# gau-nernst/llama-x

Measured on AMD Instinct MI355X. Metric: train tokens/sec Llama-3.1-8B seq4096 at 1/2/4/8 MI355X; p50 step ms, higher is better.
Workload: dtype bf16; 1 GPU; Llama-3.1-8B text-only LoRA r=16 bf16, seq=4096, 1 sequence per GPU, causal mask, base+LM head frozen (BASELINE.json configs[1]); random-init weights at 8B dimensions; seq_len=4096, parallelism=dp1, launch=hipGraph replay (fwd+bwd+AdamW), lm_head_rows=labelled only

## Files before the change

### llama-x_amd/csrc/common.h

```cpp
#pragma once
#include <hip/hip_runtime.h>
#include <stdint.h>
#include <stdarg.h>
#include <stdio.h>

#define LLX_OK 0
#define LLX_ERR_ARG -1
#define LLX_ERR_LAUNCH -2
#define LLX_ERR_UNSUPPORTED -3

void llx_set_error(const char* fmt, ...);

#define LLX_REQUIRE(cond, ...)            \
  do {                                    \
    if (!(cond)) {                        \
      llx_set_error(__VA_ARGS__);         \
      return LLX_ERR_ARG;                 \
    }                                     \
  } while (0)

#define LLX_LAUNCH_CHECK(name)                                              \
  do {                                                                      \
    hipError_t e__ = hipGetLastError();                                     \
    if (e__ != hipSuccess) {                                                \
      llx_set_error("%s: launch failed: %s", name, hipGetErrorString(e__)); \
      return LLX_ERR_LAUNCH;                                                \
    }                                                                       \
  } while (0)

typedef uint16_t bf16_t;

typedef __attribute__((ext_vector_type(8))) __bf16 bf16x8_t;
typedef __attribute__((ext_vector_type(4))) float f32x4_t;
typedef __attribute__((ext_vector_type(16))) float f32x16_t;
typedef __attribute__((ext_vector_type(4))) int i32x4_t;
typedef __attribute__((ext_vector_type(16))) int i32x16_t;
typedef __attribute__((ext_vector_type(4))) short s16x4_t;
typedef __attribute__((ext_vector_type(4))) uint32_t u32x4_t;
typedef __attribute__((ext_vector_type(2))) uint32_t u32x2_t;

#define LLX_WAVE 64

__device__ __forceinline__ float bf2f(bf16_t v) { return __uint_as_float(((uint32_t)v) << 16); }
__device__ __forceinline__ bf16_t f2bf(float f) {
  __bf16 b = (__bf16)f;
  return __builtin_bit_cast(bf16_t, b);
}
__device__ __forceinline__ uint32_t pack_bf2(float lo, float hi) {
  return (uint32_t)f2bf(lo) | ((uint32_t)f2bf(hi) << 16);
}
__device__ __forceinline__ float bflo(uint32_t w) { return __uint_as_float(w << 16); }
__device__ __forceinline__ float bfhi(uint32_t w) { return __uint_as_float(w & 0xffff0000u); }

__device__ __forceinline__ float wave_sum(float v) {
#pragma unroll
  for (int o = 32; o > 0; o >>= 1) v += __shfl_xor(v, o, 64);
  return v;
}
__device__ __forceinline__ float wave_max(float v) {
#pragma unroll
  for (int o = 32; o > 0; o >>= 1) v = fmaxf(v, __shfl_xor(v, o, 64));
  return v;
}

__device__ __forceinline__ float block_sum(float v, float* red) {
  v = wave_sum(v);
  const int lane = threadIdx.x & 63, w = threadIdx.x >> 6, nw = (blockDim.x + 63) >> 6;
  __syncthreads();
  if (lane == 0) red[w] = v;
  __syncthreads();
  float t = 0.f;
  for (int i = 0; i < nw; ++i) t += red[i];
  return t;
}
__device__ __forceinline__ float block_max(float v, float* red) {
  v = wave_max(v);
  const int lane = threadIdx.x & 63, w = threadIdx.x >> 6, nw = (blockDim.x + 63) >> 6;
  __syncthreads();
  if (lane == 0) red[w] = v;
  __syncthreads();
  float t = red[0];
  for (int i = 1; i < nw; ++i) t = fmaxf(t, red[i]);
  return t;
}

static inline int64_t cdiv64(int64_t a, int64_t b) { return (a + b - 1) / b; }

__device__ __forceinline__ float q8_absmax8(const u32x4_t& v, float amax) {
#pragma unroll
  for (int e = 0; e < 4; ++e) amax = fmaxf(amax, fmaxf(fabsf(bflo(v[e])), fabsf(bfhi(v[e]))));
  return amax;
}
__device__ __forceinline__ float q8_scale(float amax) { return amax / 127.0f; }
__device__ __forceinline__ float q8_divisor(float scale) { return fmaxf(scale, 1e-12f); }
__device__ __forceinline__ u32x2_t q8_quant8(const u32x4_t& v, float div) {
  u32x2_t o = {0u, 0u};
#pragma unroll
  for (int e = 0; e < 4; ++e) {
    const int a = (int)rintf(bflo(v[e]) / div), b = (int)rintf(bfhi(v[e]) / div);
    o[e >> 1] |= ((uint32_t)(a & 0xff) | ((uint32_t)(b & 0xff) << 8)) << ((e & 1) * 16);
  }
  return o;
}

__device__ __forceinline__ float sigmoidf_(float x) { return __builtin_amdgcn_rcpf(1.f + __expf(-x)); }
__device__ __forceinline__ u32x4_t swiglu_fwd8(const u32x4_t& gv, const u32x4_t& uv) {
  u32x4_t o;
#pragma unroll
  for (int e = 0; e < 4; ++e) {
    const float g0 = bflo(gv[e]), g1 = bfhi(gv[e]);
    const float s0 = bf2f(f2bf(g0 * sigmoidf_(g0))), s1 = bf2f(f2bf(g1 * sigmoidf_(g1)));
    o[e] = pack_bf2(s0 * bflo(uv[e]), s1 * bfhi(uv[e]));
  }
  return o;
}
__device__ __forceinline__ void swiglu_bwd8(const u32x4_t& dv, const u32x4_t& gv, const u32x4_t& uv, u32x4_t& og, u32x4_t& ou) {
#pragma unroll
  for (int e = 0; e < 4; ++e) {
    float dgs[2], dus[2];
#pragma unroll
    for (int p = 0; p < 2; ++p) {
      const float gg = p ? bfhi(gv[e]) : bflo(gv[e]);
      const float uu = p ? bfhi(uv[e]) : bflo(uv[e]);
      const float dd = p ? bfhi(dv[e]) : bflo(dv[e]);
      const float sg = sigmoidf_(gg);
      const float silu = bf2f(f2bf(gg * sg));
      dus[p] = dd * silu;
      const float ds = bf2f(f2bf(dd * uu));
      dgs[p] = ds * (sg * (1.f + gg * (1.f - sg)));
    }
    og[e] = pack_bf2(dgs[0], dgs[1]);
    ou[e] = pack_bf2(dus[0], dus[1]);
  }
}

__device__ __forceinline__ u32x4_t rope8(const u32x4_t& v, const f32x4_t& t0, const f32x4_t& t1, float sign) {
  const float cs[4] = {t0[0], t0[2], t1[0], t1[2]};
  const float sn[4] = {t0[1] * sign, t0[3] * sign, t1[1] * sign, t1[3] * sign};
  u32x4_t o;
#pragma unroll
  for (int e = 0; e < 4; ++e) {
    const float x0 = bflo(v[e]), x1 = bfhi(v[e]);
    o[e] = pack_bf2(x0 * cs[e] - x1 * sn[e], x1 * cs[e] + x0 * sn[e]);
  }
  return o;
}

__device__ __forceinline__ u32x4_t rope8(const u32x4_t& v, const float* __restrict__ tp, float sign) {
  const f32x4_t t0 = *reinterpret_cast<const f32x4_t*>(tp);
  const f32x4_t t1 = *reinterpret_cast<const f32x4_t*>(tp + 4);
  const float cs[4] = {t0[0], t0[2], t1[0], t1[2]};
  const float sn[4] = {t0[1] * sign, t0[3] * sign, t1[1] * sign, t1[3] * sign};
  u32x4_t o;
#pragma unroll
  for (int e = 0; e < 4; ++e) {
    const float x0 = bflo(v[e]), x1 = bfhi(v[e]);
    o[e] = pack_bf2(x0 * cs[e] - x1 * sn[e], x1 * cs[e] + x0 * sn[e]);
  }
  return o;
}

typedef __attribute__((ext_vector_type(8))) short llx_s16x8_t;
template <int OFF>
__device__ __forceinline__ void lds_tr_read(s16x4_t& dst, uint32_t addr) {
  asm volatile("ds_read_b64_tr_b16 %0, %1 offset:%2" : "=v"(dst) : "v"(addr), "n"(OFF));
}
__device__ __forceinline__ void lds_tr_read_rt(s16x4_t& dst, uint32_t addr, int off) {
  asm volatile("ds_read_b64_tr_b16 %0, %1 offset:%2" : "=v"(dst) : "v"(addr), "n"(off));
}
template <int N>
__device__ __forceinline__ void lds_tr_wait4(s16x4_t& a, s16x4_t& b, s16x4_t& c, s16x4_t& d) {
  asm volatile("s_waitcnt lgkmcnt(%4)" : "+v"(a), "+v"(b), "+v"(c), "+v"(d) : "n"(N));
  __builtin_amdgcn_sched_barrier(0);
}
template <int N>
__device__ __forceinline__ void lds_tr_wait8(s16x4_t (&c)[4], s16x4_t (&d)[4]) {
  asm volatile("s_waitcnt lgkmcnt(%8)" : "+v"(c[0]), "+v"(c[1]), "+v"(c[2]), "+v"(c[3]), "+v"(d[0]), "+v"(d[1]), "+v"(d[2]), "+v"(d[3]) : "n"(N));
  __builtin_amdgcn_sched_barrier(0);
}
__device__ __forceinline__ void lds_read16_rt(i32x4_t& dst, uint32_t addr, int off) {
  asm volatile("ds_read_b128 %0, %1 offset:%2" : "=v"(dst) : "v"(addr), "n"(off));
}
template <typename T>
__device__ __forceinline__ void lds_pin1(T& x) { asm volatile("" : "+v"(x)); }
template <typename T, int N>
__device__ __forceinline__ void lds_pin1(T (&x)[N]) {
#pragma unroll
  for (int i = 0; i < N; ++i) asm volatile("" : "+v"(x[i]));
}
template <typename... T>
__device__ __forceinline__ void lds_pin(T&... x) {
  (lds_pin1(x), ...);
  __builtin_amdgcn_sched_barrier(0);
}
template <int N, typename... T>
__device__ __forceinline__ void lds_wait(T&... x) {
  asm volatile("s_waitcnt lgkmcnt(%0)" : : "n"(N));
  (lds_pin1(x), ...);
  __builtin_amdgcn_sched_barrier(0);
}
__device__ __forceinline__ bf16x8_t frag_of(const s16x4_t& lo, const s16x4_t& hi) {
  const llx_s16x8_t v = {lo[0], lo[1], lo[2], lo[3], hi[0], hi[1], hi[2], hi[3]};
// ... 11 lines not shown
```

### llama-x_amd/csrc/gemm_bf16.hip

```cpp
#include "common.h"
#include <type_traits>
#include <mutex>

#define BM 256
#define BN 256
#define BK 64
#define STAGE_BYTES (2 * 256 * BK * 2)
#define A_TILE_BYTES (256 * BK * 2)
#define EPI_ROW_BYTES 528
#define GEMM_LDS_BYTES (256 * EPI_ROW_BYTES)

enum { EPI_NONE = 0, EPI_RESIDUAL = 1, EPI_BIAS = 2, EPI_BIAS_GELU = 3, EPI_COLSCALE = 4, EPI_ROWCOLSCALE = 5, EPI_SWIGLU_BWD = 6, EPI_SWIGLU_FWD = 7, EPI_ROPE = 8, EPI_SPLITK = 9, EPI_ROWCOLSCALE_F32 = 10 };

struct GemmArgs {
  const bf16_t* A; const bf16_t* B; bf16_t* C;
  const bf16_t* A2; const bf16_t* B2;
  const bf16_t* E;
  const bf16_t* E2;
  int64_t lda, ldb, ldc, lde, lda2, ldb2;
  int M, N, K, K2;
  int grid_m, grid_n;
  int col0, col_end;
  const bf16_t* sa; const bf16_t* sb;
  const float* rope;
  int rope_S, rope_cols;
  const int* m_valid;
  float* C32;
  int splits;
};

typedef __attribute__((address_space(3))) void lds_void;
typedef const __attribute__((address_space(1))) void gbl_void;

__device__ __forceinline__ float gelu_erf(float x) { return 0.5f * x * (1.0f + erff(x * 0.70710678118654752440f)); }

template <int EPI, bool I8, int PIPE, int BNT = 256>
__global__ __launch_bounds__(512, 2) void gemm_nt_kernel(const GemmArgs g) {
  static_assert(BNT == 256 || BNT == 128, "tile width");
  static_assert(PIPE == 1, "the four-phase main loop is the only one");
  static_assert(BNT == 256 || EPI != EPI_SWIGLU_FWD, "the SwiGLU-forward epilogue needs the full tile");
  constexpr int ESZ = I8 ? 1 : 2;
  constexpr int TK = 128 / ESZ;
  constexpr int WNG = BNT / 64;
  constexpr int WR = 256 / (8 / WNG);
  constexpr int MI = WR / 16;
  constexpr int MH = MI / 2;
  constexpr int BSI = BNT / 64;
  constexpr int EROW = BNT * 2 + 16;
  extern __shared__ __attribute__((aligned(16))) char smem[];
  const int tid = threadIdx.x;
  const int lane = tid & 63;
  const int wave = __builtin_amdgcn_readfirstlane(tid >> 6);
  const int wm = wave / WNG, wn = wave % WNG;

  int grid_m = g.grid_m;
  if (g.m_valid != nullptr) grid_m = min(grid_m, (*g.m_valid + BM - 1) / BM);
  const int nsplit = EPI == EPI_SPLITK ? g.splits : 1;
  const int nwg = grid_m * g.grid_n * nsplit;
  int bid = blockIdx.x;
  if (bid >= nwg) return;
  {
    const int q = nwg >> 3, r = nwg & 7, x = bid & 7;
    bid = (x < r ? x * (q + 1) : r * (q + 1) + (x - r) * q) + (bid >> 3);
  }
  const int split = EPI == EPI_SPLITK ? bid / (grid_m * g.grid_n) : 0;
  if constexpr (EPI == EPI_SPLITK) bid -= split * (grid_m * g.grid_n);
  const int GROUP_M = 4;
  const int width = GROUP_M * g.grid_n;
  const int group = bid / width;
  const int gsz = min(grid_m - group * GROUP_M, GROUP_M);
  const int pid_m = group * GROUP_M + ((bid % width) % gsz);
  const int pid_n = (bid % width) / gsz;
  constexpr bool SPLITN = EPI == EPI_SWIGLU_FWD;
  const int halfN = g.N >> 1;
  const int m0 = pid_m * BM, n0 = SPLITN ? pid_n * (BN / 2) : g.col0 + pid_n * BNT;
  auto col_of = [&](int nl) { return SPLITN ? (nl < BN / 2 ? n0 + nl : halfN + n0 + nl - BN / 2) : min(n0 + nl, g.col_end - 1); };

  const int srow = tid >> 3;
  const int schunk = (tid & 7) ^ ((tid >> 4) & 7);
  int arow[4], brow[4];
#pragma unroll
  for (int i = 0; i < 4; ++i) {
    arow[i] = min(m0 + i * 64 + srow, g.M - 1);
    brow[i] = SPLITN ? (i < 2 ? n0 + i * 64 + srow : halfN + n0 + (i - 2) * 64 + srow) : min(n0 + (i % BSI) * 64 + srow, g.col_end - 1);
  }
  const int nk1 = g.K / TK / nsplit;
  const int nk = nk1 + g.K2 / 64;
  const int kofs = split * nk1;

  uint32_t aoff[4], boff[4];
#pragma unroll
  for (int i = 0; i < 4; ++i) {
    aoff[i] = (uint32_t)((int64_t)arow[i] * g.lda * ESZ + schunk * 16);
    boff[i] = (uint32_t)((int64_t)brow[i] * g.ldb * ESZ + schunk * 16);
  }
  const __amdgpu_buffer_rsrc_t rsA = lds_dma_rsrc(g.A, (uint32_t)(((int64_t)(g.M - 1) * g.lda + g.K) * ESZ));
  const __amdgpu_buffer_rsrc_t rsB = lds_dma_rsrc(g.B, (uint32_t)(((int64_t)(g.N - 1) * g.ldb + g.K) * ESZ));

  const int frow = lane & 15;
  const int fsw = (lane >> 1) & 7;
  const int fq = lane >> 4;
  const int a_base = (wm * WR + frow) * 128;
  const int b_base = (wn * 64 + frow) * 128;
  const int slot0 = ((0 * 4 + fq) ^ fsw) * 16;
  const int slot1 = ((1 * 4 + fq) ^ fsw) * 16;
  const uint32_t sbase = (uint32_t)(uintptr_t)(__attribute__((address_space(3))) char*)smem;
  const uint32_t fa0 = sbase + a_base + slot0, fa1 = sbase + a_base + slot1;
  const uint32_t fb0 = sbase + A_TILE_BYTES + b_base + slot0, fb1 = sbase + A_TILE_BYTES + b_base + slot1;
  constexpr bool EARLY_AHI = !I8;

  using acc_t = typename std::conditional<I8, i32x4_t, f32x4_t>::type;
  acc_t acc[MI][4];
#pragma unroll
  for (int i = 0; i < MI; ++i)
#pragma unroll
    for (int j = 0; j < 4; ++j) acc[i][j] = acc_t{0, 0, 0, 0};

  auto stage_q = [&](auto steady_tag, int kt, int which) {
    constexpr bool steady = decltype(steady_tag)::value;
    if constexpr (!steady) {
      if (kt >= nk) return;
    }
    const int half = which >> 1, hi = which & 1;
    const int np = half ? BSI / 2 : 2;
    char* sT = smem + (kt & 1) * STAGE_BYTES + half * A_TILE_BYTES + hi * np * 8192;
    if (steady || kt < nk1) {
      const uint32_t koff = (uint32_t)(kt + kofs) * 128;
#pragma unroll
      for (int j = 0; j < 2; ++j) {
        if (j < np) {
          if (half) lds_dma16(rsB, (llx_lds_void*)(sT + (j * 512 + wave * 64) * 16), boff[np * hi + j], koff);
          else lds_dma16(rsA, (llx_lds_void*)(sT + (j * 512 + wave * 64) * 16), aoff[2 * hi + j], koff);
        }
      }
    } else {
      const char* base = (const char*)(half ? g.B2 : g.A2) + (int64_t)(kt - nk1) * 128;
      const int64_t l = (half ? g.ldb2 : g.lda2) * 2;
#pragma unroll
      for (int j = 0; j < 2; ++j) {
        if (j < np) {
          const char* src = base + (int64_t)(half ? brow[np * hi + j] : arow[2 * hi + j]) * l + schunk * 16;
          __builtin_amdgcn_global_load_lds((gbl_void*)src, (lds_void*)(sT + (j * 512 + wave * 64) * 16), 16, 0, 0);
        }
      }
    }
  };
  auto mfma_t = [&](auto ext_tag, const i32x4_t& b, const i32x4_t& a, acc_t& c) {
    constexpr bool ext_phase = decltype(ext_tag)::value;
    if constexpr (I8) {
      if constexpr (ext_phase) {
        f32x4_t cf = __builtin_bit_cast(f32x4_t, c);
        cf = __builtin_amdgcn_mfma_f32_16x16x32_bf16(__builtin_bit_cast(bf16x8_t, b), __builtin_bit_cast(bf16x8_t, a), cf, 0, 0, 0);
        c = __builtin_bit_cast(acc_t, cf);
      } else {
        c = __builtin_amdgcn_mfma_i32_16x16x64_i8(b, a, c, 0, 0, 0);
      }
    } else {
      c = __builtin_amdgcn_mfma_f32_16x16x32_bf16(__builtin_bit_cast(bf16x8_t, b), __builtin_bit_cast(bf16x8_t, a), c, 0, 0, 0);
    }
  };
  auto dequant_in_place = [&]() {
    if constexpr (I8) {
      float sbv[4][4], rsv[MI];
#pragma unroll
      for (int ni = 0; ni < 4; ++ni)
#pragma unroll
        for (int e = 0; e < 4; ++e) sbv[ni][e] = bf2f(g.sb[col_of(wn * 64 + ni * 16 + fq * 4 + e)]);
#pragma unroll
      for (int mi = 0; mi < MI; ++mi) rsv[mi] = bf2f(g.sa[min(m0 + wm * WR + mi * 16 + frow, g.M - 1)]);
#pragma unroll
      for (int mi = 0; mi < MI; ++mi) {
        const float rs = rsv[mi];
#pragma unroll
        for (int ni = 0; ni < 4; ++ni) {
          f32x4_t cf;
#pragma unroll
          for (int e = 0; e < 4; ++e) cf[e] = bf2f(f2bf(((float)acc[mi][ni][e] * rs) * sbv[ni][e]));
          acc[mi][ni] = __builtin_bit_cast(acc_t, cf);
        }
      }
    }
  };
  {
    const std::false_type guarded{};
    stage_q(guarded, 0, 0); stage_q(guarded, 0, 1); stage_q(guarded, 0, 2); stage_q(guarded, 0, 3);
    stage_q(guarded, 1, 2); stage_q(guarded, 1, 3); stage_q(guarded, 1, 0);
  }
  auto ktile = [&](int kt, auto ext_tag, auto steady_tag) __attribute__((always_inline)) {
    constexpr bool steady = decltype(steady_tag)::value;
    auto mfma = [&](const i32x4_t& b, const i32x4_t& a, acc_t& c) { mfma_t(ext_tag, b, a, c); };
    auto pin_acc = [&](int m_lo, int n_lo) {
#pragma unroll
      for (int m4 = 0; m4 < MH; ++m4)
#pragma unroll
        for (int n2 = 0; n2 < 2; ++n2) lds_pin1(acc[m_lo + m4][n_lo + n2]);
    };
    const uint32_t so = (uint32_t)(kt & 1) * STAGE_BYTES;
    const uint32_t pa0 = so + fa0, pa1 = so + fa1, pb0 = so + fb0, pb1 = so + fb1;
    if (steady || kt + 1 < nk) {
      if constexpr (BSI == 4) asm volatile("s_waitcnt vmcnt(6)" ::: "memory");
      else asm volatile("s_waitcnt vmcnt(4)" ::: "memory");
    } else asm volatile("s_waitcnt vmcnt(0)" ::: "memory");
    __builtin_amdgcn_s_barrier();
    asm volatile("" ::: "memory");
    stage_q(steady_tag, kt + 1, 1);
    i32x4_t bfr[2][4], af[2][MH], ah0[MH];
#pragma unroll
    for (int ks = 0; ks < 2; ++ks) {
#pragma unroll
      for (int n2 = 0; n2 < 2; ++n2) lds_read16_rt(bfr[ks][n2], ks ? pb1 : pb0, n2 * 16 * 128);
#pragma unroll
      for (int m4 = 0; m4 < MH; ++m4) lds_read16_rt(af[ks][m4], ks ? pa1 : pa0, m4 * 16 * 128);
    }
#pragma unroll
    for (int ks = 0; ks < 2; ++ks)
#pragma unroll
      for (int n2 = 0; n2 < 2; ++n2) lds_read16_rt(bfr[ks][2 + n2], ks ? pb1 : pb0, (2 + n2) * 16 * 128);
    __builtin_amdgcn_s_setprio(1);
    lds_wait<MH + 6>(bfr[0][0], bfr[0][1], af[0]);
#pragma unroll
    for (int m4 = 0; m4 < MH; ++m4)
#pragma unroll
      for (int n2 = 0; n2 < 2; ++n2) mfma(bfr[0][n2], af[0][m4], acc[m4][n2]);
    pin_acc(0, 0);
    lds_wait<4>(bfr[1][0], bfr[1][1], af[1]);
#pragma unroll
    for (int m4 = 0; m4 < MH; ++m4)
#pragma unroll
      for (int n2 = 0; n2 < 2; ++n2) mfma(bfr[1][n2], af[1][m4], acc[m4][n2]);
    __builtin_amdgcn_s_setprio(0);
    lds_wait<0>(bfr[0][2], bfr[0][3], bfr[1][2], bfr[1][3]);
    asm volatile("" ::: "memory");
    __builtin_amdgcn_s_barrier();
    asm volatile("" ::: "memory");
    stage_q(steady_tag, kt + 2, 2);
    if constexpr (EARLY_AHI) {
#pragma unroll
      for (int m4 = 0; m4 < MH; ++m4) lds_read16_rt(ah0[m4], pa0, (MH + m4) * 16 * 128);
      __builtin_amdgcn_sched_barrier(0);
    }
    __builtin_amdgcn_s_setprio(1);
#pragma unroll
    for (int ks = 0; ks < 2; ++ks)
#pragma unroll
      for (int m4 = 0; m4 < MH; ++m4)
#pragma unroll
        for (int n2 = 0; n2 < 2; ++n2) mfma(bfr[ks][2 + n2], af[ks][m4], acc[m4][2 + n2]);
    __builtin_amdgcn_s_setprio(0);
    stage_q(steady_tag, kt + 2, 3);
    pin_acc(0, 2);
    lds_pin(af[0], af[1]);
    i32x4_t (&ah)[MH] = EARLY_AHI ? ah0 : af[0];
    if constexpr (!EARLY_AHI) {
#pragma unroll
      for (int m4 = 0; m4 < MH; ++m4) lds_read16_rt(af[0][m4], pa0, (MH + m4) * 16 * 128);
    }
#pragma unroll
    for (int m4 = 0; m4 < MH; ++m4) lds_read16_rt(af[1][m4], pa1, (MH + m4) * 16 * 128);
    __builtin_amdgcn_s_setprio(1);
    lds_wait<MH>(ah);
#pragma unroll
    for (int m4 = 0; m4 < MH; ++m4)
#pragma unroll
      for (int n2 = 0; n2 < 2; ++n2) mfma(bfr[0][2 + n2], ah[m4], acc[MH + m4][2 + n2]);
    pin_acc(MH, 2);
    lds_wait<0>(af[1]);
#pragma unroll
    for (int m4 = 0; m4 < MH; ++m4)
#pragma unroll
      for (int n2 = 0; n2 < 2; ++n2) mfma(bfr[1][2 + n2], af[1][m4], acc[MH + m4][2 + n2]);
    __builtin_amdgcn_s_setprio(0);
    asm volatile("" ::: "memory");
    __builtin_amdgcn_s_barrier();
    asm volatile("" ::: "memory");
    stage_q(steady_tag, kt + 2, 0);
    __builtin_amdgcn_s_setprio(1);
#pragma unroll
    for (int ks = 0; ks < 2; ++ks)
#pragma unroll
      for (int m4 = 0; m4 < MH; ++m4)
#pragma unroll
        for (int n2 = 0; n2 < 2; ++n2) mfma(bfr[ks][n2], ks ? af[1][m4] : ah[m4], acc[MH + m4][n2]);
    __builtin_amdgcn_s_setprio(0);
  };
  const int nk_main = I8 ? nk1 : nk;
  int kt = 0;
#pragma unroll 1
  for (; kt + 2 < nk1; ++kt) ktile(kt, std::false_type{}, std::true_type{});
#pragma unroll 1
  for (; kt < nk_main; ++kt) ktile(kt, std::false_type{}, std::false_type{});
  if constexpr (I8) {
    if (nk > nk1) {
      dequant_in_place();
      for (kt = nk1; kt < nk; ++kt) ktile(kt, std::true_type{}, std::false_type{});
    }
  }
  __syncthreads();

  if constexpr (EPI == EPI_SPLITK) {
    float* P = g.C32 + (int64_t)split * g.M * g.N;
#pragma unroll
    for (int mi = 0; mi < MI; ++mi) {
      const int gm = m0 + wm * WR + mi * 16 + frow;
#pragma unroll
      for (int ni = 0; ni < 4; ++ni) {
        const int gn = n0 + wn * 64 + ni * 16 + fq * 4;
        if (gm < g.M && gn < g.col_end) *reinterpret_cast<f32x4_t*>(P + (int64_t)gm * g.N + gn) = acc[mi][ni];
      }
    }
    return;
  }
  if constexpr (EPI == EPI_ROWCOLSCALE_F32) {
    static_assert(I8, "int8 kernel only");
    float* Cf = reinterpret_cast<float*>(g.C);
    const float* saf = reinterpret_cast<const float*>(g.sa);
    const float* sbf = reinterpret_cast<const float*>(g.sb);
#pragma unroll
    for (int mi = 0; mi < MI; ++mi) {
      const int gm = m0 + wm * WR + mi * 16 + frow;
      const float rs = saf[min(gm, g.M - 1)];
#pragma unroll
      for (int ni = 0; ni < 4; ++ni) {
        const int gn = n0 + wn * 64 + ni * 16 + fq * 4;
        if (gm < g.M && gn < g.col_end) {
          const f32x4_t cs = *reinterpret_cast<const f32x4_t*>(sbf + gn);
          f32x4_t c;
#pragma unroll
          for (int e = 0; e < 4; ++e) c[e] = ((float)acc[mi][ni][e] * rs) * cs[e];
          *reinterpret_cast<f32x4_t*>(Cf + (int64_t)gm * g.ldc + gn) = c;
        }
      }
    }
    return;
  }
  constexpr int NIT = BNT / 16;
  constexpr int EB0 = (EPI == EPI_SWIGLU_BWD || EPI == EPI_ROPE) ? 4 : 8;
  constexpr int EB = EB0 < NIT / 2 ? EB0 : NIT / 2;
  constexpr bool AUX = EPI == EPI_RESIDUAL || EPI == EPI_BIAS || EPI == EPI_BIAS_GELU || EPI == EPI_SWIGLU_BWD || EPI == EPI_ROPE || EPI == EPI_COLSCALE;
  auto load_aux = [&](int it0, u32x4_t (&aux0)[EB], u32x4_t (&aux1)[EB]) {
    if constexpr (AUX) {
#pragma unroll
      for (int j = 0; j < EB; ++j) {
        const int q = (it0 + j) * 512 + tid;
        const int row = q / (BNT / 8), cc = q % (BNT / 8);
        const int gmc = min(m0 + row, g.M - 1), gnc = min(n0 + cc * 8, g.col_end - 8);
        if constexpr (EPI == EPI_RESIDUAL) {
          aux0[j] = *reinterpret_cast<const u32x4_t*>(g.E + (int64_t)gmc * g.lde + gnc);
        } else if constexpr (EPI == EPI_SWIGLU_BWD) {
          aux0[j] = *reinterpret_cast<const u32x4_t*>(g.E + (int64_t)gmc * g.lde + gnc);
          aux1[j] = *reinterpret_cast<const u32x4_t*>(g.E + (int64_t)gmc * g.lde + g.N + gnc);
        } else if constexpr (EPI == EPI_ROPE) {
          const float* tp = g.rope + ((int64_t)(gmc % g.rope_S) * 64 + ((gnc & 127) >> 1)) * 2;
          aux0[j] = *reinterpret_cast<const u32x4_t*>(tp);
          aux1[j] = *reinterpret_cast<const u32x4_t*>(tp + 4);
        } else {
          aux0[j] = *reinterpret_cast<const u32x4_t*>(g.E + gnc);
        }
      }
    }
  };
  u32x4_t auxA0[EB], auxA1[EB], auxB0[EB], auxB1[EB];
  if constexpr (!SPLITN) load_aux(0, auxA0, auxA1);
  float sbv[4][4], rsv[MI];
  if constexpr (I8) {
    if (g.K2 <= 0) {
#pragma unroll
      for (int ni = 0; ni < 4; ++ni)
#pragma unroll
        for (int e = 0; e < 4; ++e) sbv[ni][e] = bf2f(g.sb[col_of(wn * 64 + ni * 16 + fq * 4 + e)]);
#pragma unroll
      for (int mi = 0; mi < MI; ++mi) rsv[mi] = bf2f(g.sa[min(m0 + wm * WR + mi * 16 + frow, g.M - 1)]);
    }
  }
#pragma unroll
  for (int mi = 0; mi < MI; ++mi) {
    const int m = wm * WR + mi * 16 + frow;
    float rs = 1.f;
    if constexpr (I8) rs = rsv[mi];
#pragma unroll
    for (int ni = 0; ni < 4; ++ni) {
      const int n = wn * 64 + ni * 16 + fq * 4;
      float c[4];
      if constexpr (I8) {
        if (g.K2 > 0) {
          const f32x4_t cf = __builtin_bit_cast(f32x4_t, acc[mi][ni]);
#pragma unroll
          for (int e = 0; e < 4; ++e) c[e] = cf[e];
        } else {
#pragma unroll
          for (int e = 0; e < 4; ++e) c[e] = ((float)acc[mi][ni][e] * rs) * sbv[ni][e];
        }
      } else {
#pragma unroll
        for (int e = 0; e < 4; ++e) c[e] = acc[mi][ni][e];
      }
      u32x2_t pk;
      pk[0] = pack_bf2(c[0], c[1]);
      pk[1] = pack_bf2(c[2], c[3]);
      *reinterpret_cast<u32x2_t*>(smem + m * EROW + n * 2) = pk;
    }
  }
  __syncthreads();
  if constexpr (SPLITN) {
    bf16_t* H = const_cast<bf16_t*>(g.E);
#pragma unroll 4
    for (int it = 0; it < 8; ++it) {
      const int q = it * 512 + tid;
      const int row = q >> 4, cc = q & 15;
      const int gm = m0 + row, gn = n0 + cc * 8;
      if (gm < g.M) {
        const u32x4_t gv = *reinterpret_cast<const u32x4_t*>(smem + row * EPI_ROW_BYTES + cc * 16);
        const u32x4_t uv = *reinterpret_cast<const u32x4_t*>(smem + row * EPI_ROW_BYTES + (cc + 16) * 16);
        *reinterpret_cast<u32x4_t*>(g.C + (int64_t)gm * g.ldc + gn) = gv;
        *reinterpret_cast<u32x4_t*>(g.C + (int64_t)gm * g.ldc + halfN + gn) = uv;
        *reinterpret_cast<u32x4_t*>(H + (int64_t)gm * g.lde + gn) = swiglu_fwd8(gv, uv);
      }
    }
    return;
  }
  auto combine = [&](int it0, const u32x4_t (&aux0)[EB], const u32x4_t (&aux1)[EB]) {
#pragma unroll
    for (int j = 0; j < EB; ++j) {
      const int q = (it0 + j) * 512 + tid;
      const int row = q / (BNT / 8), cc = q % (BNT / 8);
      const int gm = m0 + row, gn = n0 + cc * 8;
      if (gm < g.M && gn < g.col_end) {
        u32x4_t v = *reinterpret_cast<const u32x4_t*>(smem + row * EROW + cc * 16);
        if constexpr (EPI == EPI_RESIDUAL) {
          const u32x4_t r = aux0[j];
#pragma unroll
          for (int e = 0; e < 4; ++e) v[e] = pack_bf2(bflo(v[e]) + bflo(r[e]), bfhi(v[e]) + bfhi(r[e]));
        } else if constexpr (EPI == EPI_BIAS || EPI == EPI_BIAS_GELU) {
          const u32x4_t bb = aux0[j];
#pragma unroll
          for (int e = 0; e < 4; ++e) {
            float lo = bflo(v[e]) + bflo(bb[e]), hi = bfhi(v[e]) + bfhi(bb[e]);
            if constexpr (EPI == EPI_BIAS_GELU) {
              lo = gelu_erf(bf2f(f2bf(lo)));
              hi = gelu_erf(bf2f(f2bf(hi)));
            }
            v[e] = pack_bf2(lo, hi);
          }
        } else if constexpr (EPI == EPI_SWIGLU_BWD) {
          u32x4_t og, ou;
          swiglu_bwd8(v, aux0[j], aux1[j], og, ou);
          *reinterpret_cast<u32x4_t*>(g.C + (int64_t)gm * g.ldc + g.N + gn) = ou;
          v = og;
        } else if constexpr (EPI == EPI_ROPE) {
          if (gn < g.rope_cols) v = rope8(v, __builtin_bit_cast(f32x4_t, aux0[j]), __builtin_bit_cast(f32x4_t, aux1[j]), 1.f);
        } else if constexpr (EPI == EPI_COLSCALE) {
          const u32x4_t sc = aux0[j];
#pragma unroll
          for (int e = 0; e < 4; ++e) v[e] = pack_bf2(bflo(v[e]) * bflo(sc[e]), bfhi(v[e]) * bfhi(sc[e]));
        }
        *reinterpret_cast<u32x4_t*>(g.C + (int64_t)gm * g.ldc + gn) = v;
      }
    }
  };
  static_assert((NIT / EB) % 2 == 0, "the batches alternate between two register sets");
#pragma unroll 1
  for (int it0 = 0; it0 < NIT; it0 += 2 * EB) {
    load_aux(it0 + EB, auxB0, auxB1);
    combine(it0, auxA0, auxA1);
    if (it0 + 2 * EB < NIT) load_aux(it0 + 2 * EB, auxA0, auxA1);
    combine(it0 + EB, auxB0, auxB1);
  }
}

template <int EPI, bool I8, int BNT = 256>
static int launch_gemm_p(const GemmArgs& a, hipStream_t stream) {
  auto kern = gemm_nt_kernel<EPI, I8, 1, BNT>;
  static std::once_flag attr_once;
  static hipError_t attr_err = hipSuccess;
  std::call_once(attr_once, [&] { attr_err = hipFuncSetAttribute((const void*)kern, hipFuncAttributeMaxDynamicSharedMemorySize, GEMM_LDS_BYTES); });
  if (attr_err != hipSuccess) {
    llx_set_error("llx_gemm_nt_bf16: cannot raise dynamic LDS limit: %s", hipGetErrorString(attr_err));
    return LLX_ERR_LAUNCH;
  }
  hipLaunchKernelGGL(kern, dim3(a.grid_m * a.grid_n * (EPI == EPI_SPLITK ? a.splits : 1)), dim3(512), GEMM_LDS_BYTES, stream, a);
  LLX_LAUNCH_CHECK("llx_gemm_nt_bf16");
  return LLX_OK;
}

template <int EPI, bool I8 = false>
static int launch_gemm(const GemmArgs& a, hipStream_t stream) {
  if constexpr (EPI != EPI_SWIGLU_FWD) {
    const int tiles = a.grid_m * a.grid_n, tail = tiles % 256;
    if (a.col0 == 0 && a.col_end == a.N && a.N % 256 == 0 && tiles > 256 && tail > 0 && tail <= 128 && tail % a.grid_m == 0) {
      const int tail_cols = tail / a.grid_m * 256;
      GemmArgs full = a, half = a;
      full.col_end = a.N - tail_cols;
      full.grid_n = a.grid_n - tail / a.grid_m;
      half.col0 = a.N - tail_cols;
      half.grid_n = tail_cols / 128;
      const int rc = launch_gemm_p<EPI, I8, 256>(full, stream);
      if (rc != LLX_OK) return rc;
      return launch_gemm_p<EPI, I8, 128>(half, stream);
    }
  }
  return launch_gemm_p<EPI, I8>(a, stream);
}

static GemmArgs make_args(const void* A, int64_t lda, const void* B, int64_t ldb, void* C, int64_t ldc, int64_t M, int64_t N, int64_t K) {
  GemmArgs a = {};
  a.A = (const bf16_t*)A; a.B = (const bf16_t*)B; a.C = (bf16_t*)C;
  a.lda = lda; a.ldb = ldb; a.ldc = ldc;
  a.M = (int)M; a.N = (int)N; a.K = (int)K;
  a.grid_m = (int)cdiv64(M, BM); a.grid_n = (int)cdiv64(N, BN);
  a.col_end = (int)N;
  a.splits = 1;
  return a;
}

static int check_extent(const char* who, int64_t M, int64_t N, int64_t K, int64_t lda, int64_t ldb, int esz) {
  LLX_REQUIRE(M < (1 << 30) && N < (1 << 30) && K < (1 << 30), "%s: dimension too large", who);
  LLX_REQUIRE(M * lda * esz < (int64_t)4294967296 && N * ldb * esz < (int64_t)4294967296, "%s: operand larger than 4 GiB (32-bit tile offsets)", who);
  return LLX_OK;
}

static int gemm_nt_bf16_impl(const void* A, int64_t lda, const void* B, int64_t ldb, void* C, int64_t ldc, int64_t M,
                             int64_t N, int64_t K, const void* A2, int64_t lda2, const void* B2, int64_t ldb2, int64_t K2,
                             int epilogue, const void* E, int64_t lde, const float* rope, int64_t rope_S, int64_t rope_cols,
                             hipStream_t stream, const int32_t* m_valid = nullptr) {
  LLX_REQUIRE(A && B && C, "llx_gemm_nt_bf16: null pointer");
  LLX_REQUIRE(M > 0 && N > 0 && K > 0, "llx_gemm_nt_bf16: empty problem M=%lld N=%lld K=%lld", (long long)M, (long long)N, (long long)K);
  LLX_REQUIRE(K % BK == 0 && K2 % BK == 0, "llx_gemm_nt_bf16: K=%lld and K2=%lld must be multiples of 64", (long long)K, (long long)K2);
  LLX_REQUIRE(N % 8 == 0, "llx_gemm_nt_bf16: N=%lld must be a multiple of 8", (long long)N);
  LLX_REQUIRE(lda % 8 == 0 && ldb % 8 == 0 && ldc % 8 == 0, "llx_gemm_nt_bf16: row strides must be multiples of 8 elements");
  LLX_REQUIRE(((uintptr_t)A | (uintptr_t)B | (uintptr_t)C) % 16 == 0, "llx_gemm_nt_bf16: pointers must be 16-byte aligned");
  LLX_REQUIRE(K2 == 0 || (A2 && B2 && lda2 % 8 == 0 && ldb2 % 8 == 0 && ((uintptr_t)A2 | (uintptr_t)B2) % 16 == 0),
              "llx_gemm_nt_bf16: bad K-extension operands");
  LLX_REQUIRE(epilogue == EPI_NONE || epilogue == EPI_ROPE || (E && (uintptr_t)E % 16 == 0), "llx_gemm_nt_bf16: epilogue operand missing/unaligned");
  LLX_REQUIRE(epilogue != EPI_ROPE || (rope && (uintptr_t)rope % 16 == 0 && rope_S > 0 && rope_cols >= 0 && rope_cols <= N && rope_cols % 128 == 0),
              "llx_gemm_nt_bf16_rope: need an aligned fp32 table, rope_S > 0 and rope_cols a multiple of 128 within N");
  LLX_REQUIRE((epilogue != EPI_RESIDUAL && epilogue != EPI_SWIGLU_BWD) || lde % 8 == 0, "llx_gemm_nt_bf16: residual / gate|up stride must be a multiple of 8");
  LLX_REQUIRE(epilogue != EPI_SWIGLU_BWD || (lde >= 2 * N && ldc >= 2 * N), "llx_gemm_nt_bf16: the SwiGLU-backward epilogue reads E[M,2N] (gate|up) and writes C[M,2N] (dg|du)");
  if (const int rc = check_extent("llx_gemm_nt_bf16", M, N, K, lda, ldb, 2); rc != LLX_OK) return rc;
  GemmArgs a = make_args(A, lda, B, ldb, C, ldc, M, N, K);
  a.A2 = (const bf16_t*)A2; a.B2 = (const bf16_t*)B2; a.lda2 = lda2; a.ldb2 = ldb2; a.K2 = (int)K2;
  a.E = (const bf16_t*)E; a.lde = lde;
  a.rope = rope; a.rope_S = (int)rope_S; a.rope_cols = (int)rope_cols;
  a.m_valid = m_valid;
  switch (epilogue) {
    case EPI_NONE: return launch_gemm<EPI_NONE>(a, stream);
    case EPI_RESIDUAL: return launch_gemm<EPI_RESIDUAL>(a, stream);
    case EPI_BIAS: return launch_gemm<EPI_BIAS>(a, stream);
    case EPI_BIAS_GELU: return launch_gemm<EPI_BIAS_GELU>(a, stream);
    case EPI_COLSCALE: return launch_gemm<EPI_COLSCALE>(a, stream);
    case EPI_SWIGLU_BWD: return launch_gemm<EPI_SWIGLU_BWD>(a, stream);
    case EPI_ROPE: return launch_gemm<EPI_ROPE>(a, stream);
    case EPI_SWIGLU_FWD:
      LLX_REQUIRE(N % 256 == 0 && lde % 8 == 0, "llx_gemm_nt_bf16: the SwiGLU-forward epilogue needs N = 2I with I a multiple of 128");
      a.grid_n = (int)(N / 256);
      return launch_gemm<EPI_SWIGLU_FWD>(a, stream);
    default: llx_set_error("llx_gemm_nt_bf16: unknown epilogue %d", epilogue); return LLX_ERR_UNSUPPORTED;
  }
}

extern "C" int llx_gemm_nt_bf16(const void* A, int64_t lda, const void* B, int64_t ldb, void* C, int64_t ldc, int64_t M,
                                int64_t N, int64_t K, const void* A2, int64_t lda2, const void* B2, int64_t ldb2, int64_t K2,
                                int epilogue, const void* E, int64_t lde, hipStream_t stream) {
  LLX_REQUIRE(epilogue != EPI_ROPE, "llx_gemm_nt_bf16: the RoPE epilogue is llx_gemm_nt_bf16_rope");
  return gemm_nt_bf16_impl(A, lda, B, ldb, C, ldc, M, N, K, A2, lda2, B2, ldb2, K2, epilogue, E, lde, nullptr, 0, 0, stream);
}

extern "C" int llx_gemm_nt_bf16_rows(const void* A, int64_t lda, const void* B, int64_t ldb, void* C, int64_t ldc, int64_t M,
                                     int64_t N, int64_t K, const void* A2, int64_t lda2, const void* B2, int64_t ldb2, int64_t K2,
                                     int epilogue, const void* E, int64_t lde, const int32_t* m_valid, hipStream_t stream) {
  LLX_REQUIRE(epilogue != EPI_ROPE, "llx_gemm_nt_bf16_rows: the RoPE epilogue is llx_gemm_nt_bf16_rope");
  LLX_REQUIRE(m_valid && (uintptr_t)m_valid % 4 == 0, "llx_gemm_nt_bf16_rows: m_valid must be a device int32 pointer");
  return gemm_nt_bf16_impl(A, lda, B, ldb, C, ldc, M, N, K, A2, lda2, B2, ldb2, K2, epilogue, E, lde, nullptr, 0, 0, stream, m_valid);
}

extern "C" int llx_gemm_nt_bf16_splitk(const void* A, int64_t lda, const void* B, int64_t ldb, float* partial, int64_t M, int64_t N,
                                       int64_t K, int splits, const int32_t* m_valid, hipStream_t stream) {
  LLX_REQUIRE(A && B && partial, "llx_gemm_nt_bf16_splitk: null pointer");
  LLX_REQUIRE(M > 0 && N > 0 && K > 0 && splits >= 1 && splits <= 16, "llx_gemm_nt_bf16_splitk: bad sizes");
  LLX_REQUIRE(K % ((int64_t)BK * splits) == 0, "llx_gemm_nt_bf16_splitk: K=%lld must be a multiple of 64 * splits (%d)", (long long)K, splits);
  LLX_REQUIRE(N % 8 == 0 && lda % 8 == 0 && ldb % 8 == 0, "llx_gemm_nt_bf16_splitk: N and the row strides must be multiples of 8");
  LLX_REQUIRE(((uintptr_t)A | (uintptr_t)B | (uintptr_t)partial) % 16 == 0, "llx_gemm_nt_bf16_splitk: pointers must be 16-byte aligned");
  if (const int rc = check_extent("llx_gemm_nt_bf16_splitk", M, N, K, lda, ldb, 2); rc != LLX_OK) return rc;
  LLX_REQUIRE(m_valid == nullptr || (uintptr_t)m_valid % 4 == 0, "llx_gemm_nt_bf16_splitk: m_valid must be a device int32 pointer");
  GemmArgs a = make_args(A, lda, B, ldb, nullptr, N, M, N, K);
  a.m_valid = m_valid;
  a.C32 = partial; a.splits = splits;
  return launch_gemm_p<EPI_SPLITK, false>(a, stream);
}

__global__ __launch_bounds__(256) void splitk_combine_kernel(const float* __restrict__ partial, int splits, int64_t MN, const int32_t* __restrict__ inv,
                                                             const float* __restrict__ scale, bf16_t* __restrict__ out, int64_t ldo, int N) {
  const int i = blockIdx.x, j = inv ? inv[i] : i;
  const float sc = scale ? scale[0] : 1.f;
  for (int c = threadIdx.x; c < (N >> 2); c += 256) {
    u32x2_t o = {0u, 0u};
    if (j >= 0) {
      f32x4_t v = *reinterpret_cast<const f32x4_t*>(partial + (int64_t)j * N + c * 4);
      for (int s2 = 1; s2 < splits; ++s2) {
        const f32x4_t w = *reinterpret_cast<const f32x4_t*>(partial + s2 * MN + (int64_t)j * N + c * 4);
#pragma unroll
        for (int e = 0; e < 4; ++e) v[e] += w[e];
      }
      if (scale) {
#pragma unroll
        for (int e = 0; e < 4; ++e) v[e] = bf2f(f2bf(v[e])) * sc;
      }
      o[0] = pack_bf2(v[0], v[1]);
      o[1] = pack_bf2(v[2], v[3]);
// ... 79 lines not shown
```

Baseline: 32530 tokens/s.

## Add full-tile GEMM epilogue fast path with prefetched aux loads and packed bf16 convert

Adds a fast epilogue path for GEMM tiles that lie fully in bounds. F32 outputs are written directly from registers without staging through LDS. Bf16 epilogues use precomputed pointer walks, issue all LDS reads up front with staged waits, and prefetch residual, swiglu and rope operands ahead of and during accumulator staging, all without bounds checks. pack_bf2 now uses a vector float-to-bf16 conversion, which may map to a packed convert instruction. The cost is more code paths and higher register pressure, and the ldc-size checks guard against offset overflow.

Measured after the change: 32640 tokens/s (median of 6 runs). About the same (+0.3%).

```diff
diff --git a/llama-x_amd/csrc/common.h b/llama-x_amd/csrc/common.h
--- a/llama-x_amd/csrc/common.h
+++ b/llama-x_amd/csrc/common.h
@@ -46,8 +46,11 @@
   __bf16 b = (__bf16)f;
   return __builtin_bit_cast(bf16_t, b);
 }
+typedef __attribute__((ext_vector_type(2))) float llx_f32x2_t;
+typedef __attribute__((ext_vector_type(2))) __bf16 llx_bf16x2_t;
 __device__ __forceinline__ uint32_t pack_bf2(float lo, float hi) {
-  return (uint32_t)f2bf(lo) | ((uint32_t)f2bf(hi) << 16);
+  const llx_f32x2_t v = {lo, hi};
+  return __builtin_bit_cast(uint32_t, __builtin_convertvector(v, llx_bf16x2_t));
 }
 __device__ __forceinline__ float bflo(uint32_t w) { return __uint_as_float(w << 16); }
 __device__ __forceinline__ float bfhi(uint32_t w) { return __uint_as_float(w & 0xffff0000u); }
diff --git a/llama-x_amd/csrc/gemm_bf16.hip b/llama-x_amd/csrc/gemm_bf16.hip
--- a/llama-x_amd/csrc/gemm_bf16.hip
+++ b/llama-x_amd/csrc/gemm_bf16.hip
@@ -31,6 +31,14 @@
 
 typedef __attribute__((address_space(3))) void lds_void;
 typedef const __attribute__((address_space(1))) void gbl_void;
+
+template <int I, int N, typename F>
+__device__ __forceinline__ void static_for(F&& f) {
+  if constexpr (I < N) {
+    f(std::integral_constant<int, I>{});
+    static_for<I + 1, N>(f);
+  }
+}
 
 __device__ __forceinline__ float gelu_erf(float x) { return 0.5f * x * (1.0f + erff(x * 0.70710678118654752440f)); }
 
@@ -297,6 +305,51 @@
   }
   __syncthreads();
 
+  constexpr bool F32OUT = EPI == EPI_SPLITK || EPI == EPI_ROWCOLSCALE_F32;
+  constexpr bool USES_LDE = EPI == EPI_RESIDUAL || EPI == EPI_SWIGLU_BWD || EPI == EPI_SWIGLU_FWD;
+  constexpr uint64_t LD_BYTES_MAX = 1u << 24;
+  const int64_t ldc_bytes = (EPI == EPI_SPLITK ? (int64_t)g.N : g.ldc) * (F32OUT ? 4 : 2);
+  const int64_t lde_bytes = g.lde * 2;
+  bool full_tile = __builtin_amdgcn_readfirstlane((int)(m0 + BM <= g.M) & (int)(SPLITN || n0 + BNT <= g.col_end) &
+                                                  (int)((uint64_t)ldc_bytes < LD_BYTES_MAX) &
+                                                  (int)(!USES_LDE || (uint64_t)lde_bytes < LD_BYTES_MAX)) != 0;
+#ifdef LLX_GEMM_FULL_TILE_ONLY
+  full_tile = true;
+#endif
+
+  if constexpr (F32OUT) {
+    if (full_tile) {
+      char* p = reinterpret_cast<char*>(EPI == EPI_SPLITK ? g.C32 + (int64_t)split * g.M * g.N : reinterpret_cast<float*>(g.C)) +
+                (int64_t)(m0 + wm * WR) * ldc_bytes + (int64_t)(n0 + wn * 64) * 4;
+      const uint32_t loff = __umul24((uint32_t)frow, (uint32_t)ldc_bytes) + (uint32_t)fq * 16;
+      float rs[MI];
+      f32x4_t cs[4];
+      if constexpr (EPI == EPI_ROWCOLSCALE_F32) {
+        const float* saf = reinterpret_cast<const float*>(g.sa) + m0 + wm * WR;
+        const float* sbf = reinterpret_cast<const float*>(g.sb) + n0 + wn * 64;
+#pragma unroll
+        for (int mi = 0; mi < MI; ++mi) rs[mi] = saf[mi * 16 + frow];
+#pragma unroll
+        for (int ni = 0; ni < 4; ++ni) cs[ni] = *reinterpret_cast<const f32x4_t*>(sbf + ni * 16 + fq * 4);
+      }
+#pragma unroll
+      for (int mi = 0; mi < MI; ++mi) {
+#pragma unroll
+        for (int ni = 0; ni < 4; ++ni) {
+          f32x4_t c;
+          if constexpr (EPI == EPI_ROWCOLSCALE_F32) {
+#pragma unroll
+            for (int e = 0; e < 4; ++e) c[e] = ((float)acc[mi][ni][e] * rs[mi]) * cs[ni][e];
+          } else {
+            c = __builtin_bit_cast(f32x4_t, acc[mi][ni]);
+          }
+          *reinterpret_cast<f32x4_t*>(p + loff + ni * 64) = c;
+        }
+        p += 16 * ldc_bytes;
+      }
+      return;
+    }
+  }
   if constexpr (EPI == EPI_SPLITK) {
     float* P = g.C32 + (int64_t)split * g.M * g.N;
 #pragma unroll
@@ -359,47 +412,187 @@
       }
     }
   };
+  auto stage_acc_t = [&](auto dq_tag) __attribute__((always_inline)) {
+    constexpr bool dq = decltype(dq_tag)::value;
+    float sbv[4][4], rsv[MI];
+    if constexpr (I8 && !dq) {
+#pragma unroll
+      for (int ni = 0; ni < 4; ++ni)
+#pragma unroll
+        for (int e = 0; e < 4; ++e) sbv[ni][e] = bf2f(g.sb[col_of(wn * 64 + ni * 16 + fq * 4 + e)]);
+#pragma unroll
+      for (int mi = 0; mi < MI; ++mi) rsv[mi] = bf2f(g.sa[min(m0 + wm * WR + mi * 16 + frow, g.M - 1)]);
+    }
+#pragma unroll
+    for (int mi = 0; mi < MI; ++mi) {
+      char* srow = smem + (wm * WR + mi * 16) * EROW + frow * EROW;
+#pragma unroll
+      for (int ni = 0; ni < 4; ++ni) {
+        const int n = wn * 64 + ni * 16 + fq * 4;
+        float c[4];
+        if constexpr (I8 && dq) {
+          const f32x4_t cf = __builtin_bit_cast(f32x4_t, acc[mi][ni]);
+#pragma unroll
+          for (int e = 0; e < 4; ++e) c[e] = cf[e];
+        } else if constexpr (I8) {
+#pragma unroll
+          for (int e = 0; e < 4; ++e) c[e] = ((float)acc[mi][ni][e] * rsv[mi]) * sbv[ni][e];
+        } else {
+#pragma unroll
+          for (int e = 0; e < 4; ++e) c[e] = acc[mi][ni][e];
+        }
+        u32x2_t pk;
+        pk[0] = pack_bf2(c[0], c[1]);
+        pk[1] = pack_bf2(c[2], c[3]);
+        *reinterpret_cast<u32x2_t*>(srow + n * 2) = pk;
+      }
+    }
+  };
+  auto stage_acc = [&]() __attribute__((always_inline)) {
+    if (I8 && g.K2 > 0) stage_acc_t(std::true_type{});
+    else stage_acc_t(std::false_type{});
+  };
+  auto apply_epi = [&](u32x4_t v, const u32x4_t& a0, const u32x4_t& a1, bool rot, u32x4_t& ou) __attribute__((always_inline)) -> u32x4_t {
+    if constexpr (EPI == EPI_RESIDUAL) {
+#pragma unroll
+      for (int e = 0; e < 4; ++e) v[e] = pack_bf2(bflo(v[e]) + bflo(a0[e]), bfhi(v[e]) + bfhi(a0[e]));
+    } else if constexpr (EPI == EPI_BIAS || EPI == EPI_BIAS_GELU) {
+#pragma unroll
+      for (int e = 0; e < 4; ++e) {
+        float lo = bflo(v[e]) + bflo(a0[e]), hi = bfhi(v[e]) + bfhi(a0[e]);
+        if constexpr (EPI == EPI_BIAS_GELU) {
+          lo = gelu_erf(bf2f(f2bf(lo)));
+          hi = gelu_erf(bf2f(f2bf(hi)));
+        }
+        v[e] = pack_bf2(lo, hi);
+      }
+    } else if constexpr (EPI == EPI_SWIGLU_BWD) {
+      u32x4_t og;
+      swiglu_bwd8(v, a0, a1, og, ou);
+      v = og;
+    } else if constexpr (EPI == EPI_ROPE) {
+      const u32x4_t r = rope8(v, __builtin_bit_cast(f32x4_t, a0), __builtin_bit_cast(f32x4_t, a1), 1.f);
+#pragma unroll
+      for (int e = 0; e < 4; ++e) v[e] = rot ? r[e] : v[e];
+    } else if constexpr (EPI == EPI_COLSCALE) {
+#pragma unroll
+      for (int e = 0; e < 4; ++e) v[e] = pack_bf2(bflo(v[e]) * bflo(a0[e]), bfhi(v[e]) * bfhi(a0[e]));
+    }
+    return v;
+  };
+
+  if (full_tile) {
+    constexpr int CPR = SPLITN ? 16 : BNT / 8;
+    constexpr int RS = 512 / CPR;
+    constexpr int NP = 256 / RS;
+    const int rw = wave * (64 / CPR);
+    const uint32_t rj = (uint32_t)lane / CPR, cc = (uint32_t)lane % CPR;
+    struct Walk { char* p; int64_t step; uint32_t lane; };
+    auto walk = [&](const void* base, int64_t ld_bytes, int64_t col) {
+      Walk w;
+      w.p = reinterpret_cast<char*>(const_cast<void*>(base)) + (int64_t)(m0 + rw) * ld_bytes + col * 2;
+      w.step = (int64_t)RS * ld_bytes;
+      w.lane = __umul24(rj, (uint32_t)ld_bytes) + cc * 16;
+      return w;
+    };
+    auto at = [](const Walk& w, int it) { return reinterpret_cast<u32x4_t*>(w.p + it * w.step + w.lane); };
+    const Walk wc = walk(g.C, ldc_bytes, n0);
+    const uint32_t lrow = sbase + (uint32_t)(rw * EROW) + rj * EROW + cc * 16;
+    constexpr int LG = 4;
+    static_assert((LG - 1) * RS * EROW + 256 < 65536, "ds_read_b128 offset");
+
+    if constexpr (SPLITN) {
+      const Walk wh = walk(g.E, lde_bytes, n0);
+      stage_acc();
+      __syncthreads();
+      asm volatile("" ::: "memory");
+      i32x4_t v[2 * NP];
+#pragma unroll
+      for (int it = 0; it < NP; ++it) {
+        lds_read16_rt(v[2 * it], lrow + (it / LG) * (LG * RS * EROW), (it % LG) * RS * EROW);
+        lds_read16_rt(v[2 * it + 1], lrow + (it / LG) * (LG * RS * EROW), (it % LG) * RS * EROW + 256);
+      }
+      static_for<0, NP>([&](auto ic) {
+        constexpr int it = decltype(ic)::value;
+        lds_wait<2 * NP - 2 - 2 * it>(v[2 * it], v[2 * it + 1]);
+        const u32x4_t gv = __builtin_bit_cast(u32x4_t, v[2 * it]), uv = __builtin_bit_cast(u32x4_t, v[2 * it + 1]);
+        u32x4_t* cp = at(wc, it);
+        *cp = gv;
+        *reinterpret_cast<u32x4_t*>(reinterpret_cast<char*>(cp) + (int64_t)halfN * 2) = uv;
+        *at(wh, it) = swiglu_fwd8(gv, uv);
+      });
+      return;
+    } else {
+      constexpr bool ROWAUX = EPI == EPI_RESIDUAL || EPI == EPI_SWIGLU_BWD || EPI == EPI_ROPE;
+      constexpr int NA = ROWAUX ? NP : 1;
+      constexpr int AB = !ROWAUX ? 0 : (EPI == EPI_RESIDUAL ? 8 : 4);
+      constexpr int NPRE = EPI == EPI_RESIDUAL || NP <= 8 ? NP : 8;
+      u32x4_t a0[NA], a1[NA];
+      Walk we = wc;
+      if constexpr (EPI == EPI_RESIDUAL || EPI == EPI_SWIGLU_BWD) we = walk(g.E, lde_bytes, n0);
+      uint32_t pos = 0, pos_step = 0;
+      const char* tbase = nullptr;
+      bool rot = false;
+      if constexpr (EPI == EPI_ROPE) {
+        const uint32_t S = (uint32_t)g.rope_S;
+        const uint32_t one = __builtin_amdgcn_readfirstlane(1u % S);
+        pos_step = __builtin_amdgcn_readfirstlane((uint32_t)RS % S);
+        pos = __builtin_amdgcn_readfirstlane((uint32_t)(m0 + rw) % S);
+#pragma unroll
+        for (uint32_t k = 0; k + 1 < 64 / CPR; ++k) {
+          const uint32_t nx = pos + one;
+          pos = rj > k ? (nx >= S ? nx - S : nx) : pos;
+        }
+        tbase = reinterpret_cast<const char*>(g.rope) + (cc & 15) * 32;
+        rot = n0 + (int)cc * 8 < g.rope_cols;
+      }
+      auto load_aux_full = [&](int it) __attribute__((always_inline)) {
+        if constexpr (EPI == EPI_RESIDUAL) {
+          a0[it] = *at(we, it);
+        } else if constexpr (EPI == EPI_SWIGLU_BWD) {
+          const u32x4_t* ep = at(we, it);
+          a0[it] = *ep;
+          a1[it] = *reinterpret_cast<const u32x4_t*>(reinterpret_cast<const char*>(ep) + (int64_t)g.N * 2);
+        } else if constexpr (EPI == EPI_ROPE) {
+          const char* tp = tbase + ((uint64_t)pos << 9);
+          a0[it] = *reinterpret_cast<const u32x4_t*>(tp);
+          a1[it] = *reinterpret_cast<const u32x4_t*>(tp + 16);
+          const uint32_t nx = pos + pos_step;
+          pos = nx >= (uint32_t)g.rope_S ? nx - (uint32_t)g.rope_S : nx;
+        }
+      };
+      if constexpr (EPI == EPI_BIAS || EPI == EPI_BIAS_GELU || EPI == EPI_COLSCALE)
+        a0[0] = *reinterpret_cast<const u32x4_t*>(g.E + n0 + cc * 8);
+#pragma unroll
+      for (int it = 0; it < AB; ++it) load_aux_full(it);
+      stage_acc();
+      if constexpr (ROWAUX) {
+        __builtin_amdgcn_sched_barrier(0);
+#pragma unroll
+        for (int it = AB; it < NPRE; ++it) load_aux_full(it);
+      }
+      __syncthreads();
+      asm volatile("" ::: "memory");
+      i32x4_t v[NP];
+#pragma unroll
+      for (int it = 0; it < NP; ++it) lds_read16_rt(v[it], lrow + (it / LG) * (LG * RS * EROW), (it % LG) * RS * EROW);
+      static_for<0, NP>([&](auto ic) {
+        constexpr int it = decltype(ic)::value;
+        lds_wait<NP - 1 - it>(v[it]);
+        u32x4_t ou;
+        const u32x4_t o = apply_epi(__builtin_bit_cast(u32x4_t, v[it]), a0[ROWAUX ? it : 0], a1[ROWAUX ? it : 0], rot, ou);
+        u32x4_t* cp = at(wc, it);
+        if constexpr (EPI == EPI_SWIGLU_BWD) *reinterpret_cast<u32x4_t*>(reinterpret_cast<char*>(cp) + (int64_t)g.N * 2) = ou;
+        *cp = o;
+        if constexpr (ROWAUX && it + NPRE < NP) load_aux_full(it + NPRE);
+      });
+      return;
+    }
+  }
+
   u32x4_t auxA0[EB], auxA1[EB], auxB0[EB], auxB1[EB];
   if constexpr (!SPLITN) load_aux(0, auxA0, auxA1);
-  float sbv[4][4], rsv[MI];
-  if constexpr (I8) {
-    if (g.K2 <= 0) {
-#pragma unroll
-      for (int ni = 0; ni < 4; ++ni)
-#pragma unroll
-        for (int e = 0; e < 4; ++e) sbv[ni][e] = bf2f(g.sb[col_of(wn * 64 + ni * 16 + fq * 4 + e)]);
-#pragma unroll
-      for (int mi = 0; mi < MI; ++mi) rsv[mi] = bf2f(g.sa[min(m0 + wm * WR + mi * 16 + frow, g.M - 1)]);
-    }
-  }
-#pragma unroll
-  for (int mi = 0; mi < MI; ++mi) {
-    const int m = wm * WR + mi * 16 + frow;
-    float rs = 1.f;
-    if constexpr (I8) rs = rsv[mi];
-#pragma unroll
-    for (int ni = 0; ni < 4; ++ni) {
-      const int n = wn * 64 + ni * 16 + fq * 4;
-      float c[4];
-      if constexpr (I8) {
-        if (g.K2 > 0) {
-          const f32x4_t cf = __builtin_bit_cast(f32x4_t, acc[mi][ni]);
-#pragma unroll
-          for (int e = 0; e < 4; ++e) c[e] = cf[e];
-        } else {
-#pragma unroll
-          for (int e = 0; e < 4; ++e) c[e] = ((float)acc[mi][ni][e] * rs) * sbv[ni][e];
-        }
-      } else {
-#pragma unroll
-        for (int e = 0; e < 4; ++e) c[e] = acc[mi][ni][e];
-      }
-      u32x2_t pk;
-      pk[0] = pack_bf2(c[0], c[1]);
-      pk[1] = pack_bf2(c[2], c[3]);
-      *reinterpret_cast<u32x2_t*>(smem + m * EROW + n * 2) = pk;
-    }
-  }
+  stage_acc();
   __syncthreads();
   if constexpr (SPLITN) {
     bf16_t* H = const_cast<bf16_t*>(g.E);
@@ -426,33 +619,9 @@
       const int gm = m0 + row, gn = n0 + cc * 8;
       if (gm < g.M && gn < g.col_end) {
         u32x4_t v = *reinterpret_cast<const u32x4_t*>(smem + row * EROW + cc * 16);
-        if constexpr (EPI == EPI_RESIDUAL) {
-          const u32x4_t r = aux0[j];
-#pragma unroll
-          for (int e = 0; e < 4; ++e) v[e] = pack_bf2(bflo(v[e]) + bflo(r[e]), bfhi(v[e]) + bfhi(r[e]));
-        } else if constexpr (EPI == EPI_BIAS || EPI == EPI_BIAS_GELU) {
-          const u32x4_t bb = aux0[j];
-#pragma unroll
-          for (int e = 0; e < 4; ++e) {
-            float lo = bflo(v[e]) + bflo(bb[e]), hi = bfhi(v[e]) + bfhi(bb[e]);
-            if constexpr (EPI == EPI_BIAS_GELU) {
-              lo = gelu_erf(bf2f(f2bf(lo)));
-              hi = gelu_erf(bf2f(f2bf(hi)));
-            }
-            v[e] = pack_bf2(lo, hi);
-          }
-        } else if constexpr (EPI == EPI_SWIGLU_BWD) {
-          u32x4_t og, ou;
-          swiglu_bwd8(v, aux0[j], aux1[j], og, ou);
-          *reinterpret_cast<u32x4_t*>(g.C + (int64_t)gm * g.ldc + g.N + gn) = ou;
-          v = og;
-        } else if constexpr (EPI == EPI_ROPE) {
-          if (gn < g.rope_cols) v = rope8(v, __builtin_bit_cast(f32x4_t, aux0[j]), __builtin_bit_cast(f32x4_t, aux1[j]), 1.f);
-        } else if constexpr (EPI == EPI_COLSCALE) {
-          const u32x4_t sc = aux0[j];
-#pragma unroll
-          for (int e = 0; e < 4; ++e) v[e] = pack_bf2(bflo(v[e]) * bflo(sc[e]), bfhi(v[e]) * bfhi(sc[e]));
-        }
+        u32x4_t ou;
+        v = apply_epi(v, aux0[j], aux1[j], gn < g.rope_cols, ou);
+        if constexpr (EPI == EPI_SWIGLU_BWD) *reinterpret_cast<u32x4_t*>(g.C + (int64_t)gm * g.ldc + g.N + gn) = ou;
         *reinterpret_cast<u32x4_t*>(g.C + (int64_t)gm * g.ldc + gn) = v;
       }
     }
```
